# TankMermaid/GraphAligner

Hardware: AMD Instinct MI355X
Metric: aligned Gbp/sec (whole node), 10kb ONT reads vs chr-scale GFA (higher is better)
Workload: dtype u64

## Files before the change

### graphaligner_amd/csrc/ga_lanes.h

```cpp
#pragma once
#include <stdint.h>

#include "ga_types.h"

namespace gal {

#ifdef GA_EMULATE
#define GAL_FN inline
#else
#define GAL_FN __device__ __forceinline__
#endif

#if defined(GA_STAMPS) && !defined(GA_EMULATE)
GAL_FN uint64_t lap_clock() { return __builtin_readcyclecounter(); }
#else
GAL_FN uint64_t lap_clock() { return 0; }
#endif

constexpr int W = 64;
constexpr int INF = 0x3fffffff;
constexpr uint32_t kCutoff = 200000;
constexpr int kRecBytes = 24;
constexpr int kHdrWords = 8;
constexpr uint32_t kNone = 0xffu;
// ... 323 lines not shown
		if (k + 1 < pn) loadRec6(l.rd(LY::P_NODE + (int)l.rdb(LY::X_HASH, LY::HB_ORDER + k + 1)), nxt);
		const Rec6 rec = cur;
		cur = nxt;
		const uint32_t pack = l.rd(LY::P_PACK + s);
		if ((int)(pack >> 16) > bandwidth) continue;
		const uint32_t node = l.rd(LY::P_NODE + s);
		int rc = add(node, s, rec.w[0], pack & 0xffffu);
		if (rc != GA_OK) return rc;
		const int endScore = ew_end(l.rd(LY::P_END + s));
		if (endScore > prevMin + expand) continue;
		rc = pushOut(rec, node, endScore - prevMin + 1);
		if (rc != GA_OK) return rc;
	}
	if (cn == 0) return GA_ASSERTION;
	{ const uint64_t t2 = lap_clock(); st.blaps[1] += t2 - bt; bt = t2; }
	while (heapSize > 0)
	{
		const uint32_t node = l.rd(LY::X_HEAPN);
		const int prio = (int)l.rdh(LY::X_HEAPP, 0);
		if (prio > expand) break;
		heap_pop<N>(l, heapSize);
		if (curNodes.find(l, LY::C_NODE, cn, node) >= 0) continue;
		const int ps = prevNodes.find(l, LY::P_NODE, pn, node);
		Rec6 rec;
		loadRec6(node, rec);
		const uint32_t len = rec.w[0];
		int rc = add(node, ps, len, ps >= 0 ? (l.rd(LY::P_PACK + ps) & 0xffffu) : 0u);
		if (rc != GA_OK) return rc;
		rc = pushOut(rec, node, prio + (int)len);
		if (rc != GA_OK) return rc;
	}
	st.cn = cn;
	st.totalCols = totalCols;
	{ const uint64_t t2 = lap_clock(); st.blaps[2] += t2 - bt; bt = t2; }
	return GA_OK;
}

template <int N> GAL_FN int band_order(const GaDevGraph& g, const LaneMem& m, LaneState& st)
{
	typedef Lay<N> LY;
	const Lds& l = m.lds;
	const int cn = st.cn;
	const int pn = st.pn;
	uint32_t cur[9], nxt[9];
	auto loadRec9 = [&](int s, uint32_t (&r)[9]) {
		const uint32_t* rec = g_rec(g, l.rd(LY::C_NODE + s));
#pragma unroll
		for (int i = 0; i < 9; i++) r[i] = rec[3 + i];
	};
	for (int i = 0; i < 9; i++) { cur[i] = 0; nxt[i] = 0; }
	uint64_t bt = lap_clock();
	constexpr bool kRegs = NodeRegs<N>::kOn;
	NodeRegs<N> curNodes, prevNodes;
	curNodes.load(l, LY::C_NODE, cn);
	prevNodes.load(l, LY::P_NODE, pn);
	uint64_t outAll[4] = {0, 0, 0, 0};
	uint64_t succAll = ~0ull;
	uint32_t hasPred = 0;
	bool simple = true;
	if (cn > 0) loadRec9(0, cur);
	for (int s = 0; s < cn; s++)
	{
		if (s + 1 < cn) loadRec9(s + 1, nxt);
		uint32_t rec[12];
#pragma unroll
		for (int i = 0; i < 9; i++) { rec[3 + i] = cur[i]; cur[i] = nxt[i]; }
		const uint32_t outDeg = rec[3] >> 16, inDeg = rec[3] & 0xffffu;
		if (outDeg > 4 || inDeg > 4) return GA_PUNT;
		uint32_t slots = 0, inCur = 0, inPrv = 0, nibbles = 0;
#pragma unroll
		for (uint32_t e = 0; e < 4; e++)
		{
			int x = -1, ic = -1, ip = -1;
			if (e < outDeg) x = curNodes.find(l, LY::C_NODE, cn, rec[4 + e]);
			if (e < inDeg) { ic = curNodes.find(l, LY::C_NODE, cn, rec[8 + e]); ip = prevNodes.find(l, LY::P_NODE, pn, rec[8 + e]); }
			slots |= (x < 0 ? kNone : (uint32_t)x) << (8 * e);
			nibbles |= (x < 0 ? 15u : (uint32_t)x) << (4 * e);
			inCur |= (ic < 0 ? kNone : (uint32_t)ic) << (8 * e);
			inPrv |= (ip < 0 ? kNone : (uint32_t)ip) << (8 * e);
		}
		if constexpr (kRegs)
		{
			const uint64_t field = (uint64_t)nibbles << (16 * (s & 3));
#pragma unroll
			for (int w = 0; w < 4; w++) outAll[w] |= (s >> 2) == w ? field : 0ull;
			uint32_t nOut = 0, nIn = 0, only = 15u;
#pragma unroll
			for (uint32_t e = 0; e < 4; e++)
			{
				const uint32_t x = (nibbles >> (4 * e)) & 15u;
				if (x != 15u) { nOut++; only = x; }
				if (((inCur >> (8 * e)) & 0xffu) != kNone) nIn++;
			}
			simple = simple && nOut <= 1 && nIn <= 1;
			succAll = (succAll & ~(15ull << (4 * s))) | ((uint64_t)only << (4 * s));
			hasPred |= nIn ? 1u << s : 0u;
		}
		else
		{
			l.wr(LY::C_OUT + s, slots);
			l.wrb(LY::X_ORD, LY::OB_COLOR + s, 0);
		}
		l.wr(LY::P_PACK + s, inCur);
		l.wr(LY::C_MIN + s, inPrv);
	}
	int emitted = 0;
	{ const uint64_t t2 = lap_clock(); st.blaps[3] += t2 - bt; bt = t2; }
	if constexpr (kRegs)
	{
		bool path = false;
		uint64_t along = 0;
		{
			const uint32_t heads = ~hasPred & ((1u << cn) - 1u);
			if (simple && heads != 0 && (heads & (heads - 1u)) == 0)
			{
				int v = __builtin_ctz(heads), k = 0;
				bool ended = false;
				while (k < cn && !ended)
				{
					along |= (uint64_t)v << (4 * k);
					k++;
					const int nx = (int)(succAll >> (4 * v)) & 15;
					ended = nx == 15;
					v = nx;
				}
				path = ended && k == cn;
			}
		}
#ifdef GA_EMULATE
		const bool search = !path;
#else
		const bool search = __ballot(!path) != 0;
#endif
		if (!search)
		{
			for (int k = 0; k < cn; k++) l.wrb(LY::X_ORD, LY::OB_POST + k, (uint32_t)(along >> (4 * (cn - 1 - k))) & 15u);
			{ const uint64_t t2 = lap_clock(); st.blaps[4] += t2 - bt; bt = t2; }
			return GA_OK;
		}
		uint32_t color = 0;
		uint64_t stSlot = 0, stCur = 0;
		int sp = 0, root = 0;
		while (true)
		{
			if (sp == 0)
			{
				if (root >= cn) break;
				if (((color >> (2 * root)) & 3u) == 0)
				{
					color |= 1u << (2 * root);
					stSlot = (uint64_t)root; stCur = 0;
					sp = 1;
				}
				root++;
				continue;
			}
			const int t = 4 * (sp - 1);
			const int v = (int)(stSlot >> t) & 15;
			const int c = (int)(stCur >> t) & 15;
			if (c < 4)
			{
				const uint64_t word = (v >> 2) == 0 ? outAll[0] : (v >> 2) == 1 ? outAll[1] : (v >> 2) == 2 ? outAll[2] : outAll[3];
				const uint32_t x = (uint32_t)(word >> (16 * (v & 3) + 4 * c)) & 15u;
				const uint32_t colx = x == 15u ? 2u : (color >> (2 * x)) & 3u;
				if (colx == 2) { stCur += 1ull << t; continue; }
				if (colx == 1) return GA_UNSUPPORTED_CYCLE;
				color |= 1u << (2 * x);
				stSlot = (stSlot & ~(15ull << (t + 4))) | ((uint64_t)x << (t + 4));
				stCur &= ~(15ull << (t + 4));
				sp++;
				continue;
			}
			color = (color & ~(3u << (2 * v))) | (2u << (2 * v));
			l.wrb(LY::X_ORD, LY::OB_POST + emitted, (uint32_t)v);
			emitted++;
			sp--;
			if (sp > 0) stCur += 1ull << (t - 4);
		}
	}
	else
	{
		for (int root = 0; root < cn; root++)
		{
			if (l.rdb(LY::X_ORD, LY::OB_COLOR + root) != 0) continue;
			int sp = 1;
			l.wrb(LY::X_ORD, LY::OB_COLOR + root, 1);
			l.wrb(LY::X_ORD, LY::OB_STSLOT, (uint32_t)root);
			l.wrb(LY::X_ORD, LY::OB_STCUR, 0);
			while (sp > 0)
			{
				const int v = (int)l.rdb(LY::X_ORD, LY::OB_STSLOT + sp - 1);
				const int cur = (int)l.rdb(LY::X_ORD, LY::OB_STCUR + sp - 1);
				if (cur < 4)
				{
					const uint32_t x = (l.rd(LY::C_OUT + v) >> (8 * cur)) & 0xffu;
					const uint32_t color = x == kNone ? 2u : l.rdb(LY::X_ORD, LY::OB_COLOR + (int)x);
					if (color == 2) { l.wrb(LY::X_ORD, LY::OB_STCUR + sp - 1, (uint32_t)(cur + 1)); continue; }
					if (color == 1) return GA_UNSUPPORTED_CYCLE;
					l.wrb(LY::X_ORD, LY::OB_COLOR + (int)x, 1);
					l.wrb(LY::X_ORD, LY::OB_STSLOT + sp, x);
					l.wrb(LY::X_ORD, LY::OB_STCUR + sp, 0);
					sp++;
					continue;
				}
				l.wrb(LY::X_ORD, LY::OB_COLOR + v, 2);
				l.wrb(LY::X_ORD, LY::OB_POST + emitted, (uint32_t)v);
				emitted++;
				sp--;
				if (sp > 0) l.wrb(LY::X_ORD, LY::OB_STCUR + sp - 1, l.rdb(LY::X_ORD, LY::OB_STCUR + sp - 1) + 1);
			}
		}
	}
	{ const uint64_t t2 = lap_clock(); st.blaps[4] += t2 - bt; bt = t2; }
	return GA_OK;
}

struct Col { uint64_t vp, vn; int before; };

GAL_FN void column_step(Col& c, uint64_t eq, bool noDiag, int calc)
{
	if (noDiag) eq &= ~1ull;
	const int hin = calc - c.before;
	const uint64_t neg = (uint32_t)hin >> 31, pos = (uint32_t)(-hin) >> 31;
	const uint64_t xv = eq | c.vn;
	eq |= neg;
	const uint64_t xh = (((eq & c.vp) + c.vp) ^ c.vp) | eq;
	uint64_t ph = c.vn | ~(xh | c.vp);
	uint64_t mh = c.vp & xh;
	ph = (ph << 1) | pos;
	mh = (mh << 1) | neg;
	c.vp = mh | ~(xv | ph);
	c.vn = ph & xv;
	c.before = calc;
}
GAL_FN void column_reenter(Col& c, int d)
{
	int lost = 0, p = 64;
	bool exact = false;
	uint64_t mz = ~c.vp;
	while (mz)
	{
		const int i = __builtin_ctzll(mz);
		mz &= mz - 1;
		lost += 1 + (int)((c.vn >> i) & 1);
		if (lost >= d) { p = i; exact = lost == d; break; }
	}
	const uint64_t below = p >= 64 ? ~0ull : ((1ull << p) - 1);
	const uint64_t keep = p >= 63 ? 0ull : (~0ull << (p + 1));
	c.vp = below | (c.vp & keep) | ((p < 64 && exact) ? (1ull << p) : 0ull);
	c.vn = c.vn & keep;
	c.before -= d;
}
GAL_FN void column_merge(Col& a, const Col& b)
{
	int sa = a.before, sb = b.before;
	int prev = sa < sb ? sa : sb;
	const int outBefore = prev;
	uint64_t ovp = 0, ovn = 0;
	for (int r = 0; r < 64; r++)
	{
		sa += (int)((a.vp >> r) & 1) - (int)((a.vn >> r) & 1);
		sb += (int)((b.vp >> r) & 1) - (int)((b.vn >> r) & 1);
		const int mn = sa < sb ? sa : sb;
		ovp |= (uint64_t)(mn == prev + 1) << r;
		ovn |= (uint64_t)(mn == prev - 1) << r;
		prev = mn;
	}
	a.vp = ovp; a.vn = ovn; a.before = outBefore;
}
GAL_FN int col_end(const Col& c) { return c.before + __builtin_popcountll(c.vp) - __builtin_popcountll(c.vn); }
GAL_FN int col_value(uint64_t vp, uint64_t vn, int before, int row)
{
	const uint64_t mask = row < 63 ? ~(~0ull << (row + 1)) : ~0ull;
	return before + __builtin_popcountll(vp & mask) - __builtin_popcountll(vn & mask);
}

#if defined(GA_EMULATE)
#define GAL_NT_STORE(p, v) (*(p) = (v))
#else
#define GAL_NT_STORE(p, v) __builtin_nontemporal_store((v), (p))
#endif
template <int R> GAL_FN void rec_store(const LaneMem& m, uint32_t row, const Col& c, uint32_t endWord)
{
	uint64_t* p = (uint64_t*)(m.arena + rec_off<R>(row, m.lane, m.ls));
	p[0] = c.vp; p[1] = c.vn; p[2] = (uint64_t)(uint32_t)c.before | ((uint64_t)endWord << 32);
}
template <int R> GAL_FN void rec_load(const LaneMem& m, uint32_t row, Col& c, uint32_t& endWord)
{
	const uint64_t* p = (const uint64_t*)(m.arena + rec_off<R>(row, m.lane, m.ls));
	c.vp = p[0];
	c.vn = p[1];
	const uint64_t t = p[2];
	c.before = (int)(uint32_t)t;
	endWord = (uint32_t)(t >> 32);
}
template <int R> GAL_FN void rec_load_col(const LaneMem& m, uint32_t row, Col& c)
{
	const uint64_t* p = (const uint64_t*)(m.arena + rec_off<R>(row, m.lane, m.ls));
	c.vp = p[0];
	c.vn = p[1];
	c.before = (int)((const uint32_t*)p)[4];
}

#ifndef GA_EMULATE
template <int LW> GAL_FN void stage_flush(const LaneMem& m, uint32_t chunk)
{
#ifdef GA_EXPERIMENT_NOFLUSH
	return;
#endif
	__builtin_amdgcn_wave_barrier();
	const uint32_t part = m.flushPart, g = m.flushLane;
	const bool worker = m.tid < 60;
#pragma unroll
	for (int j = 0; j < (LW + 4) / 5; j++)
	{
		const uint32_t ln = (worker && g + 5u * (uint32_t)j < (uint32_t)LW) ? g + 5u * (uint32_t)j : 0u;
		const uint64_t* sp = m.stage + ln * 25 + part * 2;
		const uint64_t a = sp[0], b = sp[1];
		const uint32_t blk0 = m.laneBlocks[2 * ln], last = m.laneBlocks[2 * ln + 1] - 1u;
		const uint32_t at16 = (blk0 + (chunk < last ? chunk : last)) * 12u + part;
		uint64_t* d = (uint64_t*)(m.arena + (uint64_t)at16 * 16);
#ifdef GA_PLAIN_ARENA_STORES
		d[0] = a; d[1] = b;
#else
		GAL_NT_STORE(d, a); GAL_NT_STORE(d + 1, b);
#endif
	}
	__builtin_amdgcn_wave_barrier();
}
GAL_FN uint32_t wave_alloc(uint32_t mine, uint32_t top, uint32_t& first)
{
	uint32_t incl = mine;
	for (int off = 1; off < 64; off <<= 1) { const uint32_t o = (uint32_t)__shfl_up((int)incl, off, 64); if ((int)(threadIdx.x & 63) >= off) incl += o; }
	first = top + incl - mine;
	return (uint32_t)__builtin_amdgcn_readlane((int)incl, 63);
}
#endif

template <int N> constexpr bool kEqInLds = NodeRegs<N>::kOn && N >= 8;
template <int N> GAL_FN uint64_t eq_from_lds(const Lds& l, int base)
{
	return (uint64_t)l.rd(Lay<N>::C_OUT + 2 * base) | ((uint64_t)l.rd(Lay<N>::C_OUT + 2 * base + 1) << 32);
}
GAL_FN uint64_t eq_for(uint64_t e0, uint64_t e1, uint64_t e2, uint64_t e3, int base)
{
	const uint64_t lo = (base & 1) ? e1 : e0, hi = (base & 1) ? e3 : e2;
	return (base & 2) ? hi : lo;
}
GAL_FN int g_base(const GaDevGraph& g, uint64_t col) { return (int)((g.seq2[col >> 4] >> ((col & 15) * 2)) & 3); }

constexpr int kStageWords64 = 25;
#ifndef GA_EMULATE
GAL_FN uint32_t wave_max(uint32_t v)
{
	for (int off = 32; off > 0; off >>= 1) { const uint32_t o = (uint32_t)__shfl_xor((int)v, off, 64); v = v > o ? v : o; }
	return v;
}
#else
GAL_FN uint32_t wave_max(uint32_t v) { return v; }
#endif

template <int N, int U, int LW = 64>
GAL_FN void fill_slice(const GaDevGraph& g, const LaneMem& m, LaneState& st, uint32_t slice, bool active, uint32_t& blockTop, uint32_t capRows, uint32_t capCols)
{
	typedef Lay<N> LY;
	const Lds& l = m.lds;
	const bool j0 = slice == 0;
	const uint64_t e0 = st.e0, e1 = st.e1, e2 = st.e2, e3 = st.e3;
	const int rawAbove = st.rawAbove;
	const int nRowsP1 = (int)st.nRows + 1;
	int ord = active ? st.cn - 1 : -1;
	int sliceMin = INF, minSlot = -1;
	uint32_t minOffset = 0;
	int status = GA_OK;
	uint32_t tick = blockTop;
	uint32_t nFirstLo = 0, nFirstHi = 0, nPend0 = 0;
	auto request = [&](int o) {
		const int s2 = o >= 0 ? (int)l.rdb(LY::X_ORD, LY::OB_POST + o) : 0;
		const uint32_t* rec2 = g_rec(g, o >= 0 ? l.rd(LY::C_NODE + s2) : 0u);
		nFirstLo = rec2[0]; nFirstHi = rec2[1];
		const uint32_t pinfo2 = o >= 0 ? l.rd(LY::C_PINFO + s2) : (kNone << 16);
		nPend0 = m.endPrev[(uint64_t)((pinfo2 >> 16) != kNone ? (pinfo2 & 0xffffu) : 0u) * m.ls];
	};
	request(ord);
	Col c; c.vp = 0; c.vn = 0; c.before = 0;
	bool exists = false;
	int doneSlot = -1;
	auto put = [&](bool on, uint32_t row, int slot, const Col& col, uint32_t endWord) {
#ifdef GA_EMULATE
		(void)slot;
		if (on) rec_store<8>(m, row, col, endWord);
#else
		(void)row;
		if (on)
		{
			uint64_t* sp = m.stage + m.lane * kStageWords64 + slot * 3;
			sp[0] = col.vp; sp[1] = col.vn; sp[2] = (uint64_t)(uint32_t)col.before | ((uint64_t)endWord << 32);
		}
#endif
	};
	auto readBack = [&](uint32_t row, Col& col, uint32_t& endWord) {
#ifndef GA_EMULATE
		__threadfence_block();
#endif
		rec_load<8>(m, row, col, endWord);
	};
#ifdef GA_EMULATE
	while (ord >= 0)
#else
	while (__ballot(ord >= 0))
#endif
	{
		const bool act = ord >= 0;
		const int s = act ? (int)l.rdb(LY::X_ORD, LY::OB_POST + ord) : 0;
		const uint32_t geo = act ? l.rd(LY::C_GEO + s) : 0u, pinfo = act ? l.rd(LY::C_PINFO + s) : (kNone << 16);
		const uint32_t inCur = act ? l.rd(LY::P_PACK + s) : 0xffffffffu, inPrv = act ? l.rd(LY::C_MIN + s) : 0xffffffffu;
		const uint32_t colBase = geo & 0xffffu, len = geo >> 16;
		const bool inPrev = (pinfo >> 16) != kNone;
		const uint32_t pbase = pinfo & 0xffffu;
		const uint64_t firstCol = ((uint64_t)nFirstHi << 32) | nFirstLo;
		const uint32_t pend0raw = nPend0;
		request(ord - 1);
		const bool aboveAlways = j0 && inPrev;
		const uint32_t* pend = m.endPrev + (uint64_t)pbase * m.ls;
		static_assert(U == 8, "a chunk is one block of 8 arena rows");
		const uint32_t nChunks = (wave_max(len) + U - 1) / U;
		const uint32_t myBlocks = act ? (len + U - 1) / U : 0u;
		uint32_t firstBlock = tick;
#ifdef GA_EMULATE
		const uint32_t allBlocks = myBlocks;
#else
		const uint32_t allBlocks = wave_alloc(myBlocks, tick, firstBlock);
#endif
		if ((uint64_t)(tick + allBlocks + 1) * U > capRows) { if (act) status = GA_CAP_ARENA; ord = -1; break; }
		const uint32_t t0 = firstBlock * U;
#ifndef GA_EMULATE
		__builtin_amdgcn_wave_barrier();
		if (m.tid < LW) { m.laneBlocks[2 * m.lane] = myBlocks ? firstBlock : (capRows >> 3) + 1u; m.laneBlocks[2 * m.lane + 1] = myBlocks ? myBlocks : 1u; }
		__builtin_amdgcn_wave_barrier();
#endif
		const uint32_t* pendSafe = (act && inPrev) ? pend : m.endPrev;
		const uint32_t* seqSafe = g.seq2 + (act ? (firstCol >> 4) : 0);
		const uint32_t sh0 = act ? (uint32_t)(firstCol & 15) * 2 : 0u;
		uint32_t pe[U];
		uint64_t bw;
#pragma unroll
		for (int i = 0; i < U; i++) pe[i] = pendSafe[(uint64_t)i * m.ls];
		bw = (uint64_t)seqSafe[0] | ((uint64_t)seqSafe[1] << 32);
		int nodeMin = INF, zero = 0, above2 = 0;
		uint32_t endWord = 0;
		const uint32_t dummyCol = capCols + 32;
		auto emit = [&](bool on, uint32_t w, int slot) {
			if (on)
			{
				const int end = col_end(c);
				endWord = ((uint32_t)end << 3) | (exists ? 4u : 0u) | ((uint32_t)(c.vn >> 63) << 1) | (uint32_t)(c.vp >> 63);
				nodeMin = end < nodeMin ? end : nodeMin;
				if (end <= sliceMin) { sliceMin = end; minSlot = s; minOffset = w; }
			}
			m.endCur[(uint64_t)(on ? colBase + w : dummyCol) * m.ls] = endWord;
			put(on, t0 + w, slot, c, endWord);
		};
		if (act)
		{
			const int pend0 = inPrev ? ew_end(pend0raw) : INF;
			int zero0 = pend0;
			bool hasIn = false;
			Col left[4];
			bool leftEx[4];
#pragma unroll
			for (int e = 0; e < 4; e++)
			{
				const uint32_t ic = (inCur >> (8 * e)) & 0xffu, ip = (inPrv >> (8 * e)) & 0xffu;
				left[e].vp = 0; left[e].vn = 0; left[e].before = 0; leftEx[e] = false;
				if (ic == kNone && ip == kNone) continue;
				hasIn = true;
				if (ic != kNone)
				{
					if ((int)ic == doneSlot) { left[e] = c; leftEx[e] = exists; }
					else
					{
						uint32_t ew;
						readBack(l.rd(LY::C_PINFO + (int)ic) + (l.rd(LY::C_GEO + (int)ic) >> 16) - 1, left[e], ew);
						leftEx[e] = ((ew >> 2) & 1) != 0;
					}
					zero0 = zero0 < left[e].before + 1 ? zero0 : left[e].before + 1;
				}
				if (ip != kNone)
				{
					const int pe1 = ew_end(l.rd(LY::P_END + (int)ip)) + 1;
					zero0 = zero0 < pe1 ? zero0 : pe1;
				}
			}
			const int base0 = (int)(bw >> sh0) & 3;
			const uint64_t eq0 = eq_for(e0, e1, e2, e3, base0);
			const bool aboveEq0 = aboveAlways || (!j0 && rawAbove == base0);
			const bool exists0 = inPrev && pend0 == zero0;
			if (!hasIn)
			{
				if (j0 && inPrev) { c.vp = ~1ull | (uint64_t)(((eq0 & 1) != 0) ? 0 : 1); c.vn = 0; c.before = pend0; exists = true; }
				else if (inPrev) { c.vp = ~0ull; c.vn = 0; c.before = pend0; exists = true; }
				else { c.vp = ~1ull; c.vn = 0; c.before = nRowsP1; exists = false; }
			}
			else
			{
				bool first = true;
#pragma unroll
				for (int e = 0; e < 4; e++)
				{
					const uint32_t ic = (inCur >> (8 * e)) & 0xffu, ip = (inPrv >> (8 * e)) & 0xffu;
					if (ic == kNone && ip == kNone) continue;
					Col x = left[e];
					uint64_t eq = eq0;
					bool leftExists = leftEx[e];
					if (ic == kNone)
					{
						x.vp = ~0ull; x.vn = 0; x.before = ew_end(l.rd(LY::P_END + (int)ip));
						leftExists = true;
						eq &= 1ull;
					}
					int calc = x.before + 1;
					if (exists0 && ip != kNone)
					{
						const int viaDiag = ew_end2(l.rd(LY::P_END + (int)ip)) + (aboveEq0 ? 0 : 1);
						calc = calc < viaDiag ? calc : viaDiag;
					}
					column_step(x, eq, !(leftExists && ip != kNone), calc);
					if (first) { c = x; first = false; } else column_merge(c, x);
				}
				exists = exists0;
				if (inPrev && c.before > pend0) { column_reenter(c, c.before - pend0); exists = true; }
			}
			zero = zero0;
			above2 = ew_end2(pend0raw);
			l.wr(LY::C_PINFO + s, t0);
		}
		for (uint32_t j = 0; j < nChunks; j++)
		{
			const uint32_t w0 = j * U;
			const uint32_t sh = (sh0 + 2 * w0) & 31u;
			uint32_t pe2[U];
			uint64_t bw2;
#pragma unroll
			for (int i = 0; i < U; i++) pe2[i] = pendSafe[(uint64_t)(w0 + U + (uint32_t)i) * m.ls];
			{ const uint32_t* q = seqSafe + (((sh0 >> 1) + w0 + U) >> 4); bw2 = (uint64_t)q[0] | ((uint64_t)q[1] << 32); }
			uint64_t eqw[U];
			if constexpr (kEqInLds<N>)
			{
#pragma unroll
				for (int i = 0; i < U; i++) eqw[i] = eq_from_lds<N>(l, (int)(bw >> (sh + 2 * i)) & 3);
			}
#pragma unroll
			for (int i = 0; i < U; i++)
			{
				const uint32_t w = w0 + (uint32_t)i;
				const bool on = act && w < len;
				if (on && w > 0)
				{
					const int base = (int)(bw >> (sh + 2 * i)) & 3;
					const uint32_t peRaw = pe[i];
					const int pv = inPrev ? ew_end(peRaw) : INF;
					const int z1 = zero + 1;
					zero = z1 < pv ? z1 : pv;
					const bool existsW = inPrev && pv == zero;
					const bool aboveEq = aboveAlways || (!j0 && rawAbove == base);
					int calc = c.before + 1;
					if (existsW) { const int viaDiag = above2 + 1 - (aboveEq ? 1 : 0); calc = calc < viaDiag ? calc : viaDiag; }
					const bool reenter = calc > pv;
					column_step(c, kEqInLds<N> ? eqw[i] : eq_for(e0, e1, e2, e3, base), !exists, reenter ? pv : calc);
					exists = reenter || existsW;
					above2 = ew_end2(peRaw);
				}
				emit(on, w, i);
			}
#ifndef GA_EMULATE
			stage_flush<LW>(m, j);
#endif
#pragma unroll
			for (int i = 0; i < U; i++) pe[i] = pe2[i];
			bw = bw2;
		}
		tick += allBlocks;
		if (act)
		{
			if (c.before != zero) { status = GA_ASSERTION; ord = -1; }
			else
			{
				l.wr(LY::C_MIN + s, (uint32_t)nodeMin);
				l.wr(LY::C_END + s, endWord);
				doneSlot = s;
				ord--;
			}
		}
	}
	blockTop = tick;
	if (active)
	{
		st.sliceMin = sliceMin; st.minSlot = minSlot; st.minOffset = minOffset;
		if (status != GA_OK) st.status = status;
	}
}

template <int N> GAL_FN void lane_begin(const GaLanesLaunch& L, const LaneMem& m, LaneState& st, uint32_t jobIndex, bool hasJob)
{
	typedef Lay<N> LY;
	st.job = jobIndex;
	st.status = hasJob ? GA_OK : GA_NOT_RUN;
	st.live = false;
	st.pn = 0; st.cn = 0; st.prevMin = 0; st.totalCols = 0; st.rowBase = 0;
	st.e0 = st.e1 = st.e2 = st.e3 = 0; st.rawAbove = 7;
	st.sliceMin = 0; st.minSlot = 0; st.minOffset = 0;
	st.nPushed = 0; st.nRun = 0; st.maxBandNodes = 0; st.kept = 0; st.nColumns = 0; st.rampUntil = 0; st.useRamp = false;
	st.nRows = 0; st.numSlices = 0; st.seedNode = 0; st.traceRows = 0; st.eq = L.eq;
	st.logCorrect = 0; st.logWrong = 0;
	for (int i = 0; i < 8; i++) st.laps[i] = 0;
	for (int i = 0; i < 5; i++) st.blaps[i] = 0;
	if (!hasJob) return;
	const GaJob job = L.jobs[jobIndex];
	st.nRows = job.n_rows;
	st.numSlices = job.n_rows / W;
	st.seedNode = job.seed_node;
	st.traceRows = job.trace_rows;
	st.eq = L.eq + (job.rows_off / W) * 5;
	st.logCorrect = L.hmm->init_correct;
	st.logWrong = L.hmm->init_wrong;
	if (st.numSlices < 4 || st.numSlices > L.max_slices) { st.status = GA_PUNT; return; }
	const uint32_t seedLen = g_rec(L.graph, job.seed_node)[2];
	if (seedLen >= kCutoff) { st.status = GA_UNSUPPORTED_BAND; return; }
	if (seedLen > L.cap_cols || seedLen > 0xffffu) { st.status = GA_CAP_COLS; return; }
	m.lds.wr(LY::P_NODE, job.seed_node);
	m.lds.wr(LY::P_END, 0u | 4u);
	m.lds.wr(LY::P_PACK, 0);
	for (uint32_t c = 0; c < seedLen; c++) m.endPrev[(uint64_t)c * m.ls] = 4u;
	st.pn = 1;
	st.live = true;
}

template <int N> GAL_FN void lane_band(const GaLanesLaunch& L, const LaneMem& m, LaneState& st, uint32_t slice)
{
	st.totalCols = 0;
	if (!st.live) return;
	if (slice >= st.numSlices) { st.live = false; return; }
	st.useRamp = st.rampUntil >= slice;
	const int bandwidth = st.useRamp ? L.ramp_bw : L.initial_bw;
	const uint64_t* e = st.eq + (uint64_t)slice * 5;
	st.e0 = e[0]; st.e1 = e[1]; st.e2 = e[2]; st.e3 = e[3];
	const uint32_t meta = (uint32_t)e[4];
	st.rawAbove = slice > 0 ? (int)((uint32_t)e[-1] & 7u) : 7;
	int rc = project_band<N>(L.graph, m, st, bandwidth);
	if (rc == GA_OK && st.totalCols > L.cap_cols) rc = GA_CAP_COLS;
	if (rc == GA_OK) rc = band_order<N>(L.graph, m, st);
	if (rc == GA_OK && (meta & 8u)) rc = GA_ASSERTION;
	if (rc != GA_OK) { st.status = rc; st.live = false; st.totalCols = 0; }
	if constexpr (kEqInLds<N>)
	{
		const Lds& l = m.lds;
#pragma unroll
		for (int k = 0; k < 4; k++) { l.wr(Lay<N>::C_OUT + 2 * k, (uint32_t)e[k]); l.wr(Lay<N>::C_OUT + 2 * k + 1, (uint32_t)(e[k] >> 32)); }
	}
}

template <int N> GAL_FN void lane_end_slice(const GaLanesLaunch& L, LaneMem& m, LaneState& st, uint32_t slice)
{
	typedef Lay<N> LY;
	if (!st.live) return;
	const Lds& l = m.lds;
	if (st.status != GA_OK) { st.live = false; return; }
	if (st.sliceMin < st.prevMin) { st.status = GA_ASSERTION; st.live = false; return; }
	st.nRun++;
	st.nColumns += st.totalCols;
	st.maxBandNodes = st.maxBandNodes > (uint32_t)st.cn ? st.maxBandNodes : (uint32_t)st.cn;
	const GaHmmTables& hmm = *L.hmm;
	const int mism = st.sliceMin - st.prevMin;
	if (mism > 64) { st.status = GA_ASSERTION; st.live = false; return; }
	const double cc = st.logCorrect + hmm.c2c, fc = st.logWrong + hmm.f2c, cf = st.logCorrect + hmm.c2f, ff = st.logWrong + hmm.f2f;
	const bool correctFromCorrect = cc >= fc;
	const bool falseFromCorrect = cf >= ff;
	const double newCorrect = (cc > fc ? cc : fc) + hmm.correct_mult[mism];
	const double newWrong = (cf > ff ? cf : ff) + hmm.wrong_mult[mism];
	const bool currentlyCorrect = newCorrect > newWrong;
	if (!correctFromCorrect) { st.live = false; return; }
	const bool rampPossible = L.ramp_bw > L.initial_bw;
	if (!currentlyCorrect && st.rampUntil < slice && rampPossible) { st.status = GA_UNSUPPORTED_RAMP; st.live = false; return; }
	const int cn = st.cn;
	uint32_t* h = m.hdr + (uint64_t)slice * kHdrWords * m.ls;
	h[0] = (uint32_t)cn; h[1 * m.ls] = st.totalCols; h[2 * m.ls] = (uint32_t)st.sliceMin; h[3 * m.ls] = (uint32_t)st.minSlot; h[4 * m.ls] = st.minOffset;
	h[5 * m.ls] = (uint32_t)((currentlyCorrect ? 1 : 0) | (falseFromCorrect ? 2 : 0));
	h[6 * m.ls] = 0;
	uint32_t* sn = m.snodes + (uint64_t)slice * 2 * N * m.ls;
	for (int k = 0; k < cn; k++)
	{
		const uint32_t node = l.rd(LY::C_NODE + k), geo = l.rd(LY::C_GEO + k);
		sn[(uint64_t)(2 * k) * m.ls] = node;
		sn[(uint64_t)(2 * k + 1) * m.ls] = l.rd(LY::C_PINFO + k);
		l.wr(LY::P_NODE + k, node);
		l.wr(LY::P_END + k, l.rd(LY::C_END + k));
		const uint32_t rel = l.rd(LY::C_MIN + k) - (uint32_t)st.sliceMin;
		if (rel > 0xffffu) { st.status = GA_PUNT; st.live = false; return; }
		l.wr(LY::P_PACK + k, (geo & 0xffffu) | (rel << 16));
	}
	st.nPushed++;
	st.logCorrect = newCorrect; st.logWrong = newWrong;
	st.pn = cn;
	st.prevMin = st.sliceMin;
	uint32_t* t = m.endPrev; m.endPrev = m.endCur; m.endCur = t;
}

#ifndef GA_EMULATE
GAL_FN uint64_t claim_cas(uint64_t* top, uint64_t cap, uint64_t bytes)
{
	unsigned long long seen = *(volatile unsigned long long*)top;
	while (seen + bytes <= cap)
	{
		const unsigned long long prev = atomicCAS((unsigned long long*)top, seen, seen + (unsigned long long)bytes);
		if (prev == seen) return seen;
		seen = prev;
	}
	return ~0ull;
}
GAL_FN bool claim_for_wave(uint64_t* top, uint64_t cap, uint64_t bytes, uint64_t& at)
{
	const uint64_t active = __ballot(1);
	const int lane = (int)(threadIdx.x & 63);
	uint64_t before = 0, total = 0;
	for (uint64_t m = active; m; m &= m - 1)
	{
		const int src = __builtin_ctzll(m);
		const uint64_t b = ((uint64_t)(uint32_t)__shfl((int)(uint32_t)(bytes >> 32), src, 64) << 32) | (uint32_t)__shfl((int)(uint32_t)bytes, src, 64);
		if (src < lane) before += b;
		total += b;
	}
	const int leader = __builtin_ctzll(active);
	uint64_t base = ~0ull;
	if (lane == leader) base = claim_cas(top, cap, total);
	base = ((uint64_t)(uint32_t)__shfl((int)(uint32_t)(base >> 32), leader, 64) << 32) | (uint32_t)__shfl((int)(uint32_t)base, leader, 64);
	if (base != ~0ull) { at = base + before; return true; }
	bool ok = false;
	for (uint64_t m = active; m; m &= m - 1)
	{
		if (lane == __builtin_ctzll(m)) { const uint64_t a = claim_cas(top, cap, bytes); if (a != ~0ull) { at = a; ok = true; } }
	}
	return ok;
}
#endif

template <int N> GAL_FN void lane_finish(const GaLanesLaunch& L, const LaneMem& m, LaneState& st, bool hasJob)
{
	typedef Lay<N> LY;
	if (!hasJob) return;
	const GaDevGraph& g = L.graph;
	const Lds& l = m.lds;
	GaJobOut out;
	out.status = st.status; out.score = 0x7fffffff; out.n_valid = 0; out.n_run = st.nRun; out.trace_len = 0; out.max_band_nodes = st.maxBandNodes;
	out.n_columns = st.nColumns; out.trace_off = 0; out.start_node = 0; out.start_offset = 0; out.start_row = 0; out.reserved2 = 0;
	out.n_node_steps = 0; out.reserved3 = 0;
	for (int i = 0; i < 8; i++) out.stamps[i] = 0;
	int status = st.status;
	uint32_t kept = st.nPushed;
	if (status == GA_OK && kept > 0)
	{
		bool ok = (m.hdr[((uint64_t)(kept - 1) * kHdrWords + 5) * m.ls] & 1u) != 0;
		while (!ok)
		{
			kept--;
			if (kept == 0) break;
			ok = (m.hdr[((uint64_t)(kept - 1) * kHdrWords + 5) * m.ls] & 2u) != 0;
		}
	}
	out.n_valid = status == GA_OK ? kept : 0;
	uint32_t len = 0, nodeSteps = 0;
	if (status == GA_OK && kept > 0)
	{
		const int big = (int)st.nRows;
		uint32_t sIdx = kept - 1;
		uint32_t nN = 0, pN = 0, curRow = 0, prvRow = 0;
		uint32_t aN = 0, aRow = 0;
		int tCN = LY::T_CN, tCB = LY::T_CB, tPN = LY::T_PN, tPB = LY::T_PB;
		auto loadHeader = [&](uint32_t sl, uint32_t& count, uint32_t& rowBase) {
			const uint32_t* h = m.hdr + (uint64_t)sl * kHdrWords * m.ls;
			count = h[0];
			rowBase = h[6 * m.ls];
		};
		auto loadTable = [&](int tn, int tb, uint32_t sl, uint32_t count) {
			const uint32_t* sn = m.snodes + (uint64_t)sl * 2 * N * m.ls;
			for (uint32_t k = 0; k < count; k += 4)
			{
				uint32_t a[8];
#pragma unroll
				for (int i = 0; i < 8; i++) a[i] = sn[(uint64_t)(2 * k + (uint32_t)i) * m.ls];
#pragma unroll
				for (int i = 0; i < 4; i++) if (k + (uint32_t)i < count) { l.wr(tn + (int)k + i, a[2 * i]); l.wr(tb + (int)k + i, a[2 * i + 1]); }
			}
		};
		auto loadTableFrom = [&](int tn, int tb, uint32_t sl, uint32_t count, uint32_t from) {
			const uint32_t* sn = m.snodes + (uint64_t)sl * 2 * N * m.ls;
			for (uint32_t k = from; k < count; k++) { const uint32_t a0 = sn[(uint64_t)(2 * k) * m.ls], a1 = sn[(uint64_t)(2 * k + 1) * m.ls]; l.wr(tn + (int)k, a0); l.wr(tb + (int)k, a1); }
		};
		struct NodeRec { uint64_t firstCol; uint32_t inDeg; uint32_t nb[4], nbLen[4]; };
		auto loadRec = [&](uint32_t n, NodeRec& nr) {
			const uint32_t* rec = g_rec(g, n);
			nr.firstCol = ((uint64_t)rec[1] << 32) | rec[0];
			nr.inDeg = rec[3] & 0xffffu;
#pragma unroll
			for (int k = 0; k < 4; k++) { nr.nb[k] = rec[8 + k]; nr.nbLen[k] = rec[12 + k]; }
		};
		loadHeader(sIdx, nN, curRow);
		if (sIdx > 0) loadHeader(sIdx - 1, pN, prvRow);
		if (sIdx > 1) loadHeader(sIdx - 2, aN, aRow);
		loadTable(tCN, tCB, sIdx, nN);
		if (sIdx > 0) loadTable(tPN, tPB, sIdx - 1, pN);
		const uint32_t* h = m.hdr + (uint64_t)sIdx * kHdrWords * m.ls;
		out.score = (int32_t)h[2 * m.ls];
		uint32_t node = l.rd(tCN + (int)h[3 * m.ls]);
		int offset = (int)h[4 * m.ls];
		uint32_t row = sIdx * W + (W - 1);
		out.start_node = node; out.start_offset = (uint32_t)offset; out.start_row = row;
		bool tracing = true;
		const bool emitRuns = L.emit_runs != 0;
		const uint32_t traceRows = st.traceRows;
		const uint32_t capRunWords = (L.cap_moves + 3) / 4 + 8;
		uint32_t nRuns = 0, runLastOff = (uint32_t)offset, runLastRow = row;
		bool started = row < traceRows;
		auto emitRun = [&](uint32_t n, uint32_t firstOff, uint32_t firstRow) {
			if (5 * (nRuns + 1) > capRunWords) { status = GA_CAP_TRACE; tracing = false; return; }
			uint32_t* d = m.moves + (uint64_t)(5 * nRuns) * m.ls;
			d[0] = n; d[1 * m.ls] = firstOff; d[2 * m.ls] = firstRow; d[3 * m.ls] = runLastOff; d[4 * m.ls] = runLastRow;
			nRuns++;
		};
		uint64_t e[4];
		auto loadEq = [&](uint32_t sl) { const uint64_t* q = st.eq + (uint64_t)sl * 5; e[0] = q[0]; e[1] = q[1]; e[2] = q[2]; e[3] = q[3]; };
		loadEq(sIdx);
		auto recordIn = [&](int tn, int tb, uint32_t count, uint32_t rowBase, uint32_t n, uint32_t off, Col& c) -> bool {
			const int sl = find_in(l, tn, (int)count, n);
			c.vp = 0; c.vn = 0; c.before = 0;
			if (sl < 0) return false;
			rec_load_col<8>(m, rowBase + l.rd(tb + sl) + off, c);
			return true;
		};
		uint32_t pack = 0;
#ifdef GA_DEBUG_SITE
		uint32_t site = 0;
#define GAL_SITE(n) site = (n)
#else
#define GAL_SITE(n)
#endif
		constexpr int kWin = Lay<N>::T_WINCOLS;
		constexpr int tWIN = Lay<N>::T_WIN;
#ifndef GAL_BURST_SLACK
#define GAL_BURST_SLACK 4
#endif
		constexpr int kBurst = kWin - GAL_BURST_SLACK;
		Col q0, q1;
		q0.vp = q0.vn = 0; q0.before = 0; q1 = q0;
		bool needSetup = true;
		uint32_t slotRow = 0, recNode = 0xffffffffu, inDeg = 0;
		uint32_t nb[4] = {0, 0, 0, 0}, nbLen[4] = {0, 0, 0, 0};
		uint64_t firstCol = 0;
		NodeRec nx = NodeRec();
		uint32_t nxNode = 0xffffffffu, nxSlotRow = 0;
		uint64_t wbases = 0;
		int wLo = 1, wHi = 0;
		bool crossed = false, xStarted = false;
		uint32_t xRowBefore = 0, xRowAfter = 0;
		uint32_t capMoves = L.cap_moves;
		uint32_t roundsLeft = 2 * L.cap_moves + 4096;
#ifndef GA_EMULATE
		asm volatile("" : "+v"(capMoves));
#endif
		auto winRead = [&](int o, Col& c) {
			const int at = tWIN + (o - wLo) * 5;
			c.vp = ((uint64_t)l.rd(at + 1) << 32) | l.rd(at);
			c.vn = ((uint64_t)l.rd(at + 3) << 32) | l.rd(at + 2);
			c.before = (int)l.rd(at + 4);
		};
		auto putMove = [&](int res, int via) {
			if (emitRuns) return;
			const uint32_t code = res == 1 ? GA_MOVE_LEFT : res == 2 ? GA_MOVE_DIAG : GA_MOVE_UP;
			pack |= (code | (res == 3 ? 0u : ((uint32_t)via << 2))) << (8 * (len & 3));
			if ((len & 3) == 3) { m.moves[(uint64_t)(len >> 2) * m.ls] = pack; pack = 0; }
// ... 435 lines not shown
```

Before: 15.55.

## Hoist flush targets, batch flush stores, and use DPP wave scans

Computes each thread's arena flush destinations once per node (flush_targets) instead of reloading laneBlocks every chunk, and batches the stage reads before the non-temporal stores with explicit sched barriers and waitcnt. Replaces the shfl-based prefix sum and max reductions with DPP row/broadcast operations plus readlane. Pending-end loads now use a compile-time LW stride in place of m.ls. The aim is less LDS traffic and instruction overhead in the per-chunk inner loop. It risks higher register pressure, and it is only correct if m.ls equals LW.

```diff
diff --git a/graphaligner_amd/csrc/ga_lanes.h b/graphaligner_amd/csrc/ga_lanes.h
--- a/graphaligner_amd/csrc/ga_lanes.h
+++ b/graphaligner_amd/csrc/ga_lanes.h
@@ -649,36 +649,75 @@
 	c.before = (int)((const uint32_t*)p)[4];
 }
 
+constexpr int kStageWords64 = 25;
 #ifndef GA_EMULATE
-template <int LW> GAL_FN void stage_flush(const LaneMem& m, uint32_t chunk)
+template <int LW> constexpr int kFlushIters = (LW + 4) / 5;
+template <int LW> GAL_FN uint32_t flush_lane(const LaneMem& m, int j)
+{
+	static_assert(4 + 5 * (kFlushIters<LW> - 2) < LW, "only a thread's last lane can lie past the wave's lanes");
+	const uint32_t g = m.tid < 60 ? m.flushLane : 0u;
+	if (j < kFlushIters<LW> - 1) return g + 5u * (uint32_t)j;
+	return g + 5u * (uint32_t)j < (uint32_t)LW ? g + 5u * (uint32_t)j : 0u;
+}
+template <int LW> struct FlushDest { uint32_t at[kFlushIters<LW>], last12[kFlushIters<LW>]; };
+template <int LW> GAL_FN void flush_targets(const LaneMem& m, FlushDest<LW>& fd)
+{
+	uint32_t blk0[kFlushIters<LW>], nblk[kFlushIters<LW>];
+#pragma unroll
+	for (int j = 0; j < kFlushIters<LW>; j++) { const uint32_t* q = m.laneBlocks + 2 * flush_lane<LW>(m, j); blk0[j] = q[0]; nblk[j] = q[1]; }
+#pragma unroll
+	for (int j = 0; j < kFlushIters<LW>; j++) { fd.at[j] = blk0[j] * 12u + m.flushPart; fd.last12[j] = (nblk[j] - 1u) * 12u; }
+}
+template <int LW> GAL_FN void stage_flush(const LaneMem& m, const FlushDest<LW>& fd, uint32_t chunk)
 {
 #ifdef GA_EXPERIMENT_NOFLUSH
 	return;
 #endif
+	constexpr int J = kFlushIters<LW>, NG = J / 4 > 0 ? J / 4 : 1;
+	const uint32_t c12 = chunk * 12u;
 	__builtin_amdgcn_wave_barrier();
-	const uint32_t part = m.flushPart, g = m.flushLane;
-	const bool worker = m.tid < 60;
-#pragma unroll
-	for (int j = 0; j < (LW + 4) / 5; j++)
-	{
-		const uint32_t ln = (worker && g + 5u * (uint32_t)j < (uint32_t)LW) ? g + 5u * (uint32_t)j : 0u;
-		const uint64_t* sp = m.stage + ln * 25 + part * 2;
-		const uint64_t a = sp[0], b = sp[1];
-		const uint32_t blk0 = m.laneBlocks[2 * ln], last = m.laneBlocks[2 * ln + 1] - 1u;
-		const uint32_t at16 = (blk0 + (chunk < last ? chunk : last)) * 12u + part;
-		uint64_t* d = (uint64_t*)(m.arena + (uint64_t)at16 * 16);
+#pragma unroll
+	for (int k = 0; k < NG; k++)
+	{
+		uint64_t a[J], b[J];
+#pragma unroll
+		for (int j = k * J / NG; j < (k + 1) * J / NG; j++)
+		{
+			const uint64_t* sp = m.stage + flush_lane<LW>(m, j) * kStageWords64 + m.flushPart * 2;
+			a[j] = sp[0]; b[j] = sp[1];
+		}
+		uint64_t* d[J];
+#pragma unroll
+		for (int j = k * J / NG; j < (k + 1) * J / NG; j++)
+		{
+			const uint32_t at16 = fd.at[j] + (c12 < fd.last12[j] ? c12 : fd.last12[j]);
+			d[j] = (uint64_t*)(m.arena + (uint64_t)at16 * 16);
+		}
+		__builtin_amdgcn_sched_barrier(0);
+		__builtin_amdgcn_s_waitcnt(0xc07f);
+#pragma unroll
+		for (int j = k * J / NG; j < (k + 1) * J / NG; j++)
+		{
 #ifdef GA_PLAIN_ARENA_STORES
-		d[0] = a; d[1] = b;
+			d[j][0] = a[j]; d[j][1] = b[j];
 #else
-		GAL_NT_STORE(d, a); GAL_NT_STORE(d + 1, b);
-#endif
+			GAL_NT_STORE(d[j], a[j]); GAL_NT_STORE(d[j] + 1, b[j]);
+#endif
+		}
+		__builtin_amdgcn_sched_barrier(0);
 	}
 	__builtin_amdgcn_wave_barrier();
 }
+#define GAL_DPP0(v, ctrl, rows) ((uint32_t)__builtin_amdgcn_update_dpp(0, (int)(v), (ctrl), (rows), 0xf, false))
 GAL_FN uint32_t wave_alloc(uint32_t mine, uint32_t top, uint32_t& first)
 {
 	uint32_t incl = mine;
-	for (int off = 1; off < 64; off <<= 1) { const uint32_t o = (uint32_t)__shfl_up((int)incl, off, 64); if ((int)(threadIdx.x & 63) >= off) incl += o; }
+	incl += GAL_DPP0(incl, 0x111, 0xf);
+	incl += GAL_DPP0(incl, 0x112, 0xf);
+	incl += GAL_DPP0(incl, 0x114, 0xf);
+	incl += GAL_DPP0(incl, 0x118, 0xf);
+	incl += GAL_DPP0(incl, 0x142, 0xa);
+	incl += GAL_DPP0(incl, 0x143, 0xc);
 	first = top + incl - mine;
 	return (uint32_t)__builtin_amdgcn_readlane((int)incl, 63);
 }
@@ -696,12 +735,17 @@
 }
 GAL_FN int g_base(const GaDevGraph& g, uint64_t col) { return (int)((g.seq2[col >> 4] >> ((col & 15) * 2)) & 3); }
 
-constexpr int kStageWords64 = 25;
 #ifndef GA_EMULATE
 GAL_FN uint32_t wave_max(uint32_t v)
 {
-	for (int off = 32; off > 0; off >>= 1) { const uint32_t o = (uint32_t)__shfl_xor((int)v, off, 64); v = v > o ? v : o; }
-	return v;
+	uint32_t o;
+	o = GAL_DPP0(v, 0x111, 0xf); v = v > o ? v : o;
+	o = GAL_DPP0(v, 0x112, 0xf); v = v > o ? v : o;
+	o = GAL_DPP0(v, 0x114, 0xf); v = v > o ? v : o;
+	o = GAL_DPP0(v, 0x118, 0xf); v = v > o ? v : o;
+	o = GAL_DPP0(v, 0x142, 0xa); v = v > o ? v : o;
+	o = GAL_DPP0(v, 0x143, 0xc); v = v > o ? v : o;
+	return (uint32_t)__builtin_amdgcn_readlane((int)v, 63);
 }
 #else
 GAL_FN uint32_t wave_max(uint32_t v) { return v; }
@@ -785,6 +829,8 @@
 		__builtin_amdgcn_wave_barrier();
 		if (m.tid < LW) { m.laneBlocks[2 * m.lane] = myBlocks ? firstBlock : (capRows >> 3) + 1u; m.laneBlocks[2 * m.lane + 1] = myBlocks ? myBlocks : 1u; }
 		__builtin_amdgcn_wave_barrier();
+		FlushDest<LW> fd;
+		flush_targets<LW>(m, fd);
 #endif
 		const uint32_t* pendSafe = (act && inPrev) ? pend : m.endPrev;
 		const uint32_t* seqSafe = g.seq2 + (act ? (firstCol >> 4) : 0);
@@ -792,7 +838,7 @@
 		uint32_t pe[U];
 		uint64_t bw;
 #pragma unroll
-		for (int i = 0; i < U; i++) pe[i] = pendSafe[(uint64_t)i * m.ls];
+		for (int i = 0; i < U; i++) pe[i] = pendSafe[i * LW];
 		bw = (uint64_t)seqSafe[0] | ((uint64_t)seqSafe[1] << 32);
 		int nodeMin = INF, zero = 0, above2 = 0;
 		uint32_t endWord = 0;
@@ -888,8 +934,11 @@
 			const uint32_t sh = (sh0 + 2 * w0) & 31u;
 			uint32_t pe2[U];
 			uint64_t bw2;
-#pragma unroll
-			for (int i = 0; i < U; i++) pe2[i] = pendSafe[(uint64_t)(w0 + U + (uint32_t)i) * m.ls];
+			{
+				const uint32_t* pendChunk = pendSafe + (uint64_t)w0 * LW;
+#pragma unroll
+				for (int i = 0; i < U; i++) pe2[i] = pendChunk[(U + i) * LW];
+			}
 			{ const uint32_t* q = seqSafe + (((sh0 >> 1) + w0 + U) >> 4); bw2 = (uint64_t)q[0] | ((uint64_t)q[1] << 32); }
 			uint64_t eqw[U];
 			if constexpr (kEqInLds<N>)
@@ -921,7 +970,7 @@
 				emit(on, w, i);
 			}
 #ifndef GA_EMULATE
-			stage_flush<LW>(m, j);
+			stage_flush<LW>(m, fd, j);
 #endif
 #pragma unroll
 			for (int i = 0; i < U; i++) pe[i] = pe2[i];
```

New measurement: 16.35 (median of 5 runs). +5.1%, better.
